# jianwang-mpi/GlobalEgoMocap

Hardware: AMD Instinct MI355X
Metric: optimised windows/sec (10-frame, 15-joint) (higher is better)
Workload: dtype f32

## Files before the change

### globalegomocap_amd/csrc/lbfgs.hip

```cpp
#include "gem_internal.h"

namespace gem {

typedef float f32x4 __attribute__((ext_vector_type(4)));

enum { PH_INIT = 0, PH_BRACKET = 1, PH_ZOOM = 2, PH_DONE = 3 };
static_assert(PH_DONE == 3, "Workspace::done_phase (gem_internal.h) names this value for the fused compaction of gemm_rows.h");

struct AdvArgs {
    LbfgsState* state;
    const double* f;
    double* trace;
    const float* gnew;
    float *x, *d, *g, *gp, *bg0, *bg1, *trial, *S, *Y;
    uint16_t* trial_b;
    int* phase_arr;
    const int* slot_of;
    int *next_perm, *next_slot_of, *next_count;
    SlabSrc gslab;
    unsigned long long* clk;
    int Dp, hist_cap;
    gem_lbfgs_opts o;
};

__device__ __forceinline__ double cubic_interpolate(double x1, double f1, double g1, double x2, double f2, double g2,
                                                    bool has_bounds, double lo, double hi) {
    if (!has_bounds) {
        lo = x1 <= x2 ? x1 : x2;
        hi = x1 <= x2 ? x2 : x1;
    }
    const double d1 = g1 + g2 - 3.0 * (f1 - f2) / (x1 - x2);
    const double d2s = d1 * d1 - g1 * g2;
    if (d2s >= 0.0) {
        const double d2 = sqrt(d2s);
        double m;
        if (x1 <= x2) m = x2 - (x2 - x1) * ((g2 + d2 - d1) / (g2 - g1 + 2.0 * d2));
        else m = x1 - (x1 - x2) * ((g1 + d2 - d1) / (g1 - g2 + 2.0 * d2));
        double r = (m > lo) ? m : lo;
        if (!(m == m)) r = m;
        double q = (r < hi) ? r : hi;
        if (!(r == r)) q = r;
        return q;
    }
    return (lo + hi) / 2.0;
}

template <int NT>
struct BlockRed {
    double* red;
    int parity;
    __device__ __forceinline__ double sum(double v) {
        double w[1] = {v};
        sumN<1>(w);
        return w[0];
    }
    template <int N>
    __device__ __forceinline__ void sumN(double (&v)[N]) {
#pragma unroll
        for (int n = 0; n < N; ++n) v[n] = wave_sum_dpp(v[n]);
        if (NT == 64) return;
        double* r = red + 12 * parity;
        parity ^= 1;
        if ((threadIdx.x & 63) == 0) {
#pragma unroll
            for (int n = 0; n < N; ++n) r[(threadIdx.x >> 6) * 3 + n] = v[n];
        }
        __syncthreads();
#pragma unroll
        for (int n = 0; n < N; ++n) v[n] = r[n] + r[3 + n] + r[6 + n] + r[9 + n];
    }
    __device__ __forceinline__ double max(double v) {
        v = wave_max_dpp(v);
        if (NT == 64) return v;
        double* r = red + 12 * parity;
        parity ^= 1;
        if ((threadIdx.x & 63) == 0) r[(threadIdx.x >> 6) * 3] = v;
        __syncthreads();
        return nan_max(nan_max(nan_max(r[0], r[3]), r[6]), r[9]);
    }
};

template <int EPT, int NT, bool FULL, bool HB>
__device__ __forceinline__ void lbfgs_advance_body(const AdvArgs& a) {
    __shared__ double red[24];
    __shared__ double ro_s[MAX_HIST];
    __shared__ double cadj_s[MAX_HIST];
    __shared__ double al_s[MAX_HIST];
    const int b = blockIdx.x, tid = threadIdx.x;
    LbfgsState* sp = a.state + b;
    int phase = sp->phase;
    const int gslot = a.slot_of ? a.slot_of[b] : b;
    const double f_new = a.f[b];
    if (phase == PH_DONE) return;
    BlockRed<NT> R{red, 0};
#ifdef GEM_LB_PROBE
    unsigned long long ts[10];
#pragma unroll
    for (int i = 0; i < 10; ++i) ts[i] = 0ull;
#define LB_PROBE(n) do { if (a.clk) ts[n] = wall_clock64(); } while (0)
#else
#define LB_PROBE(n) do { } while (0)
#endif
    LB_PROBE(0);
    const int hmask = a.hist_cap - 1;
    const gem_lbfgs_opts& o = a.o;
    const int Dp = a.Dp;
    const size_t off = (size_t)b * Dp;

    int n_iter = sp->n_iter, evals = sp->evals, ls_iter = sp->ls_iter, ls_evals = sp->ls_evals, max_ls = sp->max_ls;
    int first_bracket = sp->first_bracket, ls_done = sp->ls_done, insuf = sp->insuf, low = sp->low, high = sp->high;
    int hist_count = sp->hist_count, hist_start = sp->hist_start;
    double loss = sp->loss, prev_loss = sp->prev_loss, t = sp->t, gtd = sp->gtd, d_norm = sp->d_norm, H_diag = sp->H_diag;
    double t_prev = sp->t_prev, f_prev = sp->f_prev, gtd_prev = sp->gtd_prev;
    double br_t[2] = {sp->br_t[0], sp->br_t[1]}, br_f[2] = {sp->br_f[0], sp->br_f[1]};
    double br_gtd[2] = {sp->br_gtd[0], sp->br_gtd[1]};
    static_assert(MAX_HIST <= NT, "one ring scalar per thread");

    if (a.trace && tid == 0) a.trace[b] = f_new;
    if (f_new != f_new && tid == 0) sp->nan_seen = 1;
    const float* gsrc = a.gnew + (size_t)gslot * Dp;
    float gn[EPT], xv[EPT], dv[EPT], gcur[EPT], yv[EPT], sv[EPT];
    bool have_x = false, have_d = false;
#pragma unroll
    for (int i = 0; i < EPT; ++i) xv[i] = dv[i] = gcur[i] = yv[i] = sv[i] = 0.f;
    auto load = [&](const float* p, float (&v)[EPT]) {
        if constexpr (EPT % 4 == 0) {
#pragma unroll
            for (int i = 0; i < EPT / 4; ++i) {
                const int e = (tid + NT * i) * 4;
                f32x4 w = {0.f, 0.f, 0.f, 0.f};
                if (FULL || e < Dp) w = *reinterpret_cast<const f32x4*>(p + off + e);
                v[4 * i] = w[0]; v[4 * i + 1] = w[1]; v[4 * i + 2] = w[2]; v[4 * i + 3] = w[3];
            }
        } else {
#pragma unroll
            for (int i = 0; i < EPT; ++i) { const int e = tid + NT * i; v[i] = (FULL || e < Dp) ? p[off + e] : 0.f; }
        }
    };
    auto store = [&](float* p, const float (&v)[EPT]) {
        if constexpr (EPT % 4 == 0) {
#pragma unroll
            for (int i = 0; i < EPT / 4; ++i) {
                const int e = (tid + NT * i) * 4;
                const f32x4 w = {v[4 * i], v[4 * i + 1], v[4 * i + 2], v[4 * i + 3]};
                if (FULL || e < Dp) *reinterpret_cast<f32x4*>(p + off + e) = w;
            }
        } else {
#pragma unroll
            for (int i = 0; i < EPT; ++i) { const int e = tid + NT * i; if (FULL || e < Dp) p[off + e] = v[i]; }
        }
    };
    auto hload = [&](const float* base, int slot, float (&v)[EPT]) {
        const size_t eo = ((size_t)b * a.hist_cap + slot) * Dp;
        if constexpr (!HB) { load(base + eo - off, v); }
        else {
            const uint16_t* q = reinterpret_cast<const uint16_t*>(base) + eo;
            if constexpr (EPT % 4 == 0) {
#pragma unroll
                for (int i = 0; i < EPT / 4; ++i) {
                    const int e = (tid + NT * i) * 4;
                    typedef unsigned int u2 __attribute__((ext_vector_type(2)));
                    u2 w = {0u, 0u};
                    if (FULL || e < Dp) w = *reinterpret_cast<const u2*>(q + e);
                    v[4 * i] = __builtin_bit_cast(float, w[0] << 16); v[4 * i + 1] = __builtin_bit_cast(float, w[0] & 0xFFFF0000u);
                    v[4 * i + 2] = __builtin_bit_cast(float, w[1] << 16); v[4 * i + 3] = __builtin_bit_cast(float, w[1] & 0xFFFF0000u);
                }
            } else {
#pragma unroll
                for (int i = 0; i < EPT; ++i) { const int e = tid + NT * i; v[i] = (FULL || e < Dp) ? __builtin_bit_cast(float, (unsigned)q[e] << 16) : 0.f; }
            }
        }
    };
    auto hstore = [&](float* base, int slot, const float (&v)[EPT]) {
        const size_t eo = ((size_t)b * a.hist_cap + slot) * Dp;
        if constexpr (!HB) { store(base + eo - off, v); }
        else {
            uint16_t* q = reinterpret_cast<uint16_t*>(base) + eo;
            if constexpr (EPT % 4 == 0) {
#pragma unroll
                for (int i = 0; i < EPT / 4; ++i) {
                    const int e = (tid + NT * i) * 4;
                    typedef __bf16 bf4 __attribute__((ext_vector_type(4)));
                    const bf4 w = __builtin_convertvector(f32x4{v[4 * i], v[4 * i + 1], v[4 * i + 2], v[4 * i + 3]}, bf4);
                    if (FULL || e < Dp) *reinterpret_cast<bf4*>(q + e) = w;
                }
            } else {
#pragma unroll
                for (int i = 0; i < EPT; ++i) { const int e = tid + NT * i; if (FULL || e < Dp) q[e] = (uint16_t)(__builtin_bit_cast(unsigned int, (float)(__bf16)v[i]) >> 16); }
            }
        }
    };
    auto store_trial = [&](const float (&v)[EPT]) {
        if (!a.trial_b) store(a.trial, v);
        if (a.trial_b) {
            uint16_t* p = a.trial_b + off;
            if constexpr (EPT % 4 == 0) {
#pragma unroll
                for (int i = 0; i < EPT / 4; ++i) {
                    const int e = (tid + NT * i) * 4;
                    typedef __bf16 bf4 __attribute__((ext_vector_type(4)));
                    const bf4 w = __builtin_convertvector(f32x4{v[4 * i], v[4 * i + 1], v[4 * i + 2], v[4 * i + 3]}, bf4);
                    if (FULL || e < Dp) *reinterpret_cast<bf4*>(p + e) = w;
                }
            } else {
#pragma unroll
                for (int i = 0; i < EPT; ++i) {
                    const int e = tid + NT * i;
                    if (FULL || e < Dp) p[e] = (uint16_t)(__builtin_bit_cast(unsigned int, (float)(__bf16)v[i]) >> 16);
                }
            }
        }
    };
    auto copy = [&](float* dst, const float* src) {
        float tmp[EPT];
        load(src, tmp);
        store(dst, tmp);
    };
    auto dot = [&](const float (&u)[EPT], const float (&v)[EPT]) {
        float p = 0.f;
#pragma unroll
        for (int i = 0; i < EPT; ++i) p += u[i] * v[i];
        return R.sum((double)p);
    };
    auto maxabs = [&](const float (&u)[EPT], float scale) {
        float p = 0.f;
#pragma unroll
        for (int i = 0; i < EPT; ++i) { const float w = fabsf(u[i] * scale); p = (w > p || w != w) ? w : p; }
        return R.max((double)p);
    };
    LB_PROBE(1);
    double ro_v = 0.0, cadj_v = 0.0;
    auto request_rest = [&]() {
        if (tid < a.hist_cap) { ro_v = sp->ro[tid]; cadj_v = sp->cadj[tid]; }
        if (phase != PH_INIT) { load(a.d, dv); load(a.x, xv); have_d = have_x = true; }
    };
    if (a.gslab.base) {
        int nslab;
        size_t stride;
        slab_layout(a.gslab, nslab, stride);
        const float* gs = a.gslab.base + (size_t)gslot * Dp;
#pragma unroll
        for (int i = 0; i < EPT; ++i) gn[i] = 0.f;
        for (int z0 = 0; z0 < nslab; z0 += 8) {
            float t[8][EPT];
#pragma unroll
            for (int k = 0; k < 8; ++k) load(gs + (size_t)min(z0 + k, nslab - 1) * stride - off, t[k]);
            if (z0 == 0) request_rest();
#pragma unroll
            for (int k = 0; k < 8; ++k)
                if (z0 + k < nslab) {
#pragma unroll
                    for (int i = 0; i < EPT; ++i) gn[i] += t[k][i];
                }
        }
        if (nslab <= 0) request_rest();
    } else {
        load(gsrc - off, gn);
        request_rest();
    }
    if (tid < a.hist_cap) { ro_s[tid] = ro_v; cadj_s[tid] = cadj_v; }
    __syncthreads();
    float* BG[2] = {a.bg0, a.bg1};

    bool do_zoom_head = false, do_ls_end = false, do_start_iter = false, finished = false, emit = false;
    bool have_ys = false;

    LB_PROBE(2);
    if (phase == PH_INIT) {
        loss = f_new;
        evals = 1;
        n_iter = 0;
        store(a.g, gn);
#pragma unroll
        for (int i = 0; i < EPT; ++i) gcur[i] = gn[i];
        if (maxabs(gn, 1.f) <= o.tol_grad) finished = true;
        else do_start_iter = true;
    } else {
        const double gtd_new = dot(gn, dv);
        if (phase == PH_BRACKET) {
            if (!first_bracket) ls_iter++;
            first_bracket = 0;
            bool enter_zoom = false;
            if (ls_iter < max_ls) {
                const bool c1 = f_new > (loss + o.c1 * t * gtd) || (ls_iter > 1 && f_new >= f_prev);
                const bool c2 = fabs(gtd_new) <= -o.c2 * gtd;
                const bool c3 = gtd_new >= 0.0;
                if (c1 || (!c2 && c3)) {
                    br_t[0] = t_prev; br_t[1] = t;
                    br_f[0] = f_prev; br_f[1] = f_new;
                    br_gtd[0] = gtd_prev; br_gtd[1] = gtd_new;
                    copy(a.bg0, a.gp);
                    store(a.bg1, gn);
                    ls_done = 0;
                    enter_zoom = true;
                } else if (c2) {
                    br_t[0] = br_t[1] = t;
                    br_f[0] = br_f[1] = f_new;
                    br_gtd[0] = br_gtd[1] = gtd_new;
                    store(a.bg0, gn);
                    ls_done = 1;
                    enter_zoom = true;
                } else {
                    const double lo_b = t + 0.01 * (t - t_prev), hi_b = t * 10.0;
                    const double t_next = cubic_interpolate(t_prev, f_prev, gtd_prev, t, f_new, gtd_new, true, lo_b, hi_b);
                    t_prev = t; f_prev = f_new; gtd_prev = gtd_new;
                    store(a.gp, gn);
                    t = t_next;
                    emit = true;
                }
            } else {
                br_t[0] = 0.0; br_t[1] = t;
                br_f[0] = loss; br_f[1] = f_new;
                br_gtd[0] = gtd; br_gtd[1] = gtd_new;
                copy(a.bg0, a.g);
                store(a.bg1, gn);
                ls_done = 0;
                enter_zoom = true;
            }
            if (enter_zoom) {
                insuf = 0;
                if (br_f[0] <= br_f[1]) { low = 0; high = 1; } else { low = 1; high = 0; }
                do_zoom_head = true;
            }
        } else {
            ls_iter++;
            if (f_new > (loss + o.c1 * t * gtd) || f_new >= br_f[low]) {
                br_t[high] = t; br_f[high] = f_new; br_gtd[high] = gtd_new;
                store(BG[high], gn);
                if (br_f[0] <= br_f[1]) { low = 0; high = 1; } else { low = 1; high = 0; }
            } else {
                if (fabs(gtd_new) <= -o.c2 * gtd) {
                    ls_done = 1;
                } else if (gtd_new * (br_t[high] - br_t[low]) >= 0.0) {
                    br_t[high] = br_t[low]; br_f[high] = br_f[low]; br_gtd[high] = br_gtd[low];
                    copy(BG[high], BG[low]);
                }
                br_t[low] = t; br_f[low] = f_new; br_gtd[low] = gtd_new;
                store(BG[low], gn);
            }
            do_zoom_head = true;
        }
    }

    LB_PROBE(3);
    if (do_zoom_head) {
        if (ls_done || ls_iter >= max_ls) {
            do_ls_end = true;
        } else if (fabs(br_t[1] - br_t[0]) * d_norm < o.ls_tol_change) {
            do_ls_end = true;
        } else {
            double tn = cubic_interpolate(br_t[0], br_f[0], br_gtd[0], br_t[1], br_f[1], br_gtd[1], false, 0.0, 0.0);
            const double hi = br_t[0] > br_t[1] ? br_t[0] : br_t[1];
            const double lo = br_t[0] > br_t[1] ? br_t[1] : br_t[0];
            const double eps = 0.1 * (hi - lo);
            const double m1 = hi - tn, m2 = tn - lo;
            if ((m1 < m2 ? m1 : m2) < eps) {
                if (insuf || tn >= hi || tn <= lo) {
                    tn = (fabs(tn - hi) < fabs(tn - lo)) ? hi - eps : lo + eps;
                    insuf = 0;
                } else {
                    insuf = 1;
                }
            } else {
                insuf = 0;
            }
            t = tn;
            phase = PH_ZOOM;
            emit = true;
        }
    }

    LB_PROBE(4);
    if (do_ls_end) {
        __syncthreads();
        t = br_t[low];
        loss = br_f[low];
        float bl[EPT], gold[EPT];
        load(BG[low], bl);
        load(a.g, gold);
        const float tf = (float)t;
#pragma unroll
        for (int i = 0; i < EPT; ++i) {
            xv[i] = xv[i] + tf * dv[i];
            yv[i] = bl[i] - gold[i];
            sv[i] = dv[i] * tf;
            gcur[i] = bl[i];
        }
        store(a.x, xv);
        store(a.g, bl);
        evals += ls_evals;
        const double gmax = maxabs(bl, 1.f);
        const double dmax = maxabs(sv, 1.f);
        if (n_iter == o.max_iter || evals >= o.max_eval || gmax <= o.tol_grad || dmax <= o.tol_change ||
            fabs(loss - prev_loss) < o.tol_change) {
            finished = true;
        } else {
            do_start_iter = true;
            have_ys = true;
        }
    }

    LB_PROBE(5);
    bool full_path = false;
    if (do_start_iter) {
        n_iter++;
        if (n_iter == 1) {
#pragma unroll
            for (int i = 0; i < EPT; ++i) dv[i] = -gcur[i];
            H_diag = 1.0;
        } else {
            (void)have_ys;
            auto ring_slot = [&](int k) { return (hist_start + k) & hmask; };
            float sprev[EPT];
            const bool has_prev = hist_count >= 1;
            if (has_prev) hload(a.S, ring_slot(hist_count - 1), sprev);
            double r3[3] = {0.0, 0.0, 0.0};
            {
                float p0 = 0.f, p1 = 0.f, p2 = 0.f;
#pragma unroll
                for (int i = 0; i < EPT; ++i) {
                    p0 += yv[i] * sv[i];
                    p1 += yv[i] * yv[i];
                    if (has_prev) p2 += sprev[i] * yv[i];
                }
                r3[0] = (double)p0; r3[1] = (double)p1; r3[2] = (double)p2;
            }
            R.template sumN<3>(r3);
            full_path = true;
            LB_PROBE(6);
            const double ys = r3[0];
            const int limit = o.history < a.hist_cap ? o.history : a.hist_cap;
            if (ys > 1e-10) {
                const int prev_slot = (hist_start + hist_count - 1) & hmask;
                if (hist_count == limit) {
                    hist_start = (hist_start + 1) & hmask;
                    hist_count--;
                }
                const int slot = (hist_start + hist_count) & hmask;
                hstore(a.Y, slot, yv);
                hstore(a.S, slot, sv);
                const bool link = has_prev && hist_count >= 1;
                hist_count++;
                H_diag = ys / r3[1];
                if (tid == 0) {
                    ro_s[slot] = 1.0 / ys; sp->ro[slot] = 1.0 / ys;
                    if (link) { cadj_s[prev_slot] = r3[2]; sp->cadj[prev_slot] = r3[2]; }
                }
                __syncthreads();
            }
            float q[EPT];
#pragma unroll
            for (int i = 0; i < EPT; ++i) q[i] = -gcur[i];
            const int hc = hist_count, np2 = (hc + 1) / 2;
            float sXa[EPT], yXa[EPT], sXb[EPT], yXb[EPT], sZa[EPT], yZa[EPT], sZb[EPT], yZb[EPT];
            auto clampk = [&](int k) { return k < 0 ? 0 : (k >= hc ? hc - 1 : k); };
            auto ld2 = [&](int kA, int kB, float (&sA)[EPT], float (&yA)[EPT], float (&sB)[EPT], float (&yB)[EPT]) {
                hload(a.S, ring_slot(clampk(kA)), sA); hload(a.Y, ring_slot(clampk(kA)), yA);
                hload(a.S, ring_slot(clampk(kB)), sB); hload(a.Y, ring_slot(clampk(kB)), yB);
            };
            auto dstep1 = [&](int kA, float (&sA)[EPT], float (&yA)[EPT], float (&sB)[EPT], float (&yB)[EPT]) {
                const int kB = kA - 1;
                const bool vB = kB >= 0;
                const int slA = (hist_start + kA) & hmask, slB = (hist_start + clampk(kB)) & hmask;
                double r2[2];
                {
                    float pa = 0.f, pb = 0.f;
#pragma unroll
                    for (int i = 0; i < EPT; ++i) { pa += sA[i] * q[i]; pb += sB[i] * q[i]; }
                    r2[0] = (double)pa; r2[1] = (double)pb;
                }
                R.template sumN<2>(r2);
                const double alA = r2[0] * ro_s[slA];
                const double alB = vB ? (r2[1] - (double)(float)alA * cadj_s[slB]) * ro_s[slB] : 0.0;
                if (tid == 0) { al_s[kA] = alA; if (vB) al_s[kB] = alB; }
                const float fa = (float)alA, fb = (float)alB;
#pragma unroll
                for (int i = 0; i < EPT; ++i) q[i] -= fa * yA[i] + fb * yB[i];
            };
            auto dstep2 = [&](int kA, float (&sA)[EPT], float (&yA)[EPT], float (&sB)[EPT], float (&yB)[EPT]) {
                const int kB = kA + 1;
                const bool vB = kB < hc;
                const int slA = (hist_start + kA) & hmask, slB = (hist_start + clampk(kB)) & hmask;
                double r2[2];
                {
                    float pa = 0.f, pb = 0.f;
#pragma unroll
                    for (int i = 0; i < EPT; ++i) { pa += yA[i] * q[i]; pb += yB[i] * q[i]; }
                    r2[0] = (double)pa; r2[1] = (double)pb;
                }
                R.template sumN<2>(r2);
                const float cfA = (float)(al_s[kA] - r2[0] * ro_s[slA]);
                const float cfB = vB ? (float)(al_s[clampk(kB)] - (r2[1] + (double)cfA * cadj_s[slA]) * ro_s[slB]) : 0.f;
#pragma unroll
                for (int i = 0; i < EPT; ++i) q[i] += cfA * sA[i] + cfB * sB[i];
            };
            if (hc > 0) ld2(hc - 1, hc - 2, sXa, yXa, sXb, yXb);
            for (int p2 = 0; p2 < np2; p2 += 2) {
                const int kA = hc - 1 - 2 * p2;
                ld2(kA - 2, kA - 3, sZa, yZa, sZb, yZb);
                dstep1(kA, sXa, yXa, sXb, yXb);
                ld2(kA - 4, kA - 5, sXa, yXa, sXb, yXb);
                if (p2 + 1 < np2) dstep1(kA - 2, sZa, yZa, sZb, yZb);
            }
            __syncthreads();
            const float hd = (float)H_diag;
#pragma unroll
            for (int i = 0; i < EPT; ++i) q[i] *= hd;
            if (hc > 0) ld2(0, 1, sXa, yXa, sXb, yXb);
            for (int p2 = 0; p2 < np2; p2 += 2) {
                const int kA = 2 * p2;
                ld2(kA + 2, kA + 3, sZa, yZa, sZb, yZb);
                dstep2(kA, sXa, yXa, sXb, yXb);
                ld2(kA + 4, kA + 5, sXa, yXa, sXb, yXb);
                if (p2 + 1 < np2) dstep2(kA + 2, sZa, yZa, sZb, yZb);
            }
#pragma unroll
            for (int i = 0; i < EPT; ++i) dv[i] = q[i];
        }
        LB_PROBE(7);
        have_d = true;
        store(a.d, dv);
        prev_loss = loss;
        if (n_iter == 1) {
            float p = 0.f;
#pragma unroll
            for (int i = 0; i < EPT; ++i) p += fabsf(gcur[i]);
            const double l1 = R.sum((double)p);
            const double inv = 1.0 / l1;
            t = (inv < 1.0 ? inv : 1.0) * o.lr;
        } else {
            t = o.lr;
        }
        gtd = dot(gcur, dv);
        if (gtd > -o.tol_change) {
            finished = true;
        } else {
            d_norm = maxabs(dv, 1.f);
            max_ls = o.max_eval - evals;
            ls_iter = 0;
            ls_evals = 0;
            t_prev = 0.0; f_prev = loss; gtd_prev = gtd;
            store(a.gp, gcur);
            phase = PH_BRACKET;
            first_bracket = 1;
            emit = true;
        }
    }

    LB_PROBE(8);
    if (finished) {
        phase = PH_DONE;
        if (!have_x) load(a.x, xv);
        store_trial(xv);
    } else if (emit) {
        if (!have_x) load(a.x, xv);
        if (!have_d) load(a.d, dv);
        const float tf = (float)t;
        float tr[EPT];
#pragma unroll
        for (int i = 0; i < EPT; ++i) tr[i] = xv[i] + tf * dv[i];
        store_trial(tr);
        ls_evals++;
    }
    if (tid == 0) {
        if (a.next_count && phase != PH_DONE) {
            const int slot = atomicAdd(a.next_count, 1);
            a.next_perm[slot] = b;
            a.next_slot_of[b] = slot;
        }
        if (a.phase_arr) a.phase_arr[b] = phase;
        sp->phase = phase; sp->n_iter = n_iter; sp->evals = evals; sp->ls_iter = ls_iter; sp->ls_evals = ls_evals;
        sp->max_ls = max_ls; sp->first_bracket = first_bracket; sp->ls_done = ls_done; sp->insuf = insuf;
        sp->low = low; sp->high = high; sp->hist_count = hist_count; sp->hist_start = hist_start;
        sp->loss = loss; sp->prev_loss = prev_loss; sp->t = t; sp->gtd = gtd; sp->d_norm = d_norm; sp->H_diag = H_diag;
        sp->t_prev = t_prev; sp->f_prev = f_prev; sp->gtd_prev = gtd_prev;
        sp->br_t[0] = br_t[0]; sp->br_t[1] = br_t[1]; sp->br_f[0] = br_f[0]; sp->br_f[1] = br_f[1];
        sp->br_gtd[0] = br_gtd[0]; sp->br_gtd[1] = br_gtd[1];
    }
    LB_PROBE(9);
#ifdef GEM_LB_PROBE
    if (a.clk && tid == 0 && full_path) {
        unsigned long long prev = ts[0];
#pragma unroll
        for (int i = 1; i < 10; ++i)
            if (ts[i]) { atomicAdd(a.clk + i, ts[i] - prev); prev = ts[i]; }
        atomicAdd(a.clk + 30, (unsigned long long)hist_count);
        atomicAdd(a.clk + 31, 1ull);
    }
#endif
    (void)full_path;
#undef LB_PROBE
}

template <int EPT, bool FULL, bool HB = false>
__global__ __launch_bounds__(256) void lbfgs_advance_kernel(AdvArgs a) { lbfgs_advance_body<EPT, 256, FULL, HB>(a); }

__global__ void lbfgs_init_kernel(LbfgsState* st, int* __restrict__ phase_arr, const float* __restrict__ trial, float* __restrict__ x, int B,
                                  int Dp) {
    const size_t i = (size_t)blockIdx.x * blockDim.x + threadIdx.x;
    if (i < (size_t)B * Dp) x[i] = trial[i];
    if (i < (size_t)B) {
        phase_arr[i] = PH_INIT;
        LbfgsState* s = st + i;
        s->phase = PH_INIT; s->n_iter = 0; s->evals = 0; s->ls_iter = 0; s->ls_evals = 0; s->max_ls = 0;
        s->first_bracket = 0; s->ls_done = 0; s->insuf = 0; s->low = 0; s->high = 1; s->hist_count = 0; s->hist_start = 0;
        s->nan_seen = 0;
        s->loss = 0; s->prev_loss = 0; s->t = 0; s->gtd = 0; s->d_norm = 0; s->H_diag = 1;
        s->t_prev = 0; s->f_prev = 0; s->gtd_prev = 0;
        s->br_t[0] = s->br_t[1] = 0; s->br_f[0] = s->br_f[1] = 0; s->br_gtd[0] = s->br_gtd[1] = 0;
    }
}

__global__ void lbfgs_stats_kernel(const LbfgsState* st, gem_window_stats* out, int B) {
    const int i = blockIdx.x * blockDim.x + threadIdx.x;
    if (i >= B) return;
    out[i].n_iter = st[i].n_iter;
    out[i].func_evals = st[i].evals;
    out[i].final_loss = (float)st[i].loss;
    out[i].status = (st[i].phase == PH_DONE ? 1 : 0) | (st[i].nan_seen ? 2 : 0);
}

static AdvArgs make_args(gem_handle* h, const gem_lbfgs_opts& o) {
    Workspace& w = h->ws;
    AdvArgs a;
    a.state = w.state; a.f = w.f; a.gnew = w.dz;
    a.trace = (w.round >= 0 && w.round < TRACE_ROUNDS) ? w.trace + (size_t)w.round * w.Bmax : nullptr;
    a.x = w.x; a.d = w.d; a.g = w.g; a.gp = w.gp; a.bg0 = w.bg0; a.bg1 = w.bg1; a.trial = w.trial; a.S = w.S; a.Y = w.Y;
    a.trial_b = h->precision == GEM_PRECISION_BF16 ? w.trial_b : nullptr;
    a.phase_arr = w.phase;
    a.slot_of = w.dyn ? w.slot_of : nullptr;
    a.next_perm = w.dyn ? w.next_perm : nullptr; a.next_slot_of = w.dyn ? w.next_slot_of : nullptr; a.next_count = w.dyn ? w.next_count : nullptr;
    a.gslab = w.dyn ? w.grad_slab : SlabSrc{};
    a.clk = w.lbfgs_clk;
    a.Dp = h->Dp; a.hist_cap = w.hist_cap; a.o = o;
    return a;
}

int launch_lbfgs_init(gem_handle* h, int B, const gem_lbfgs_opts& o, hipStream_t s) {
    (void)o;
    const size_t n = (size_t)B * h->Dp;
    hipLaunchKernelGGL(lbfgs_init_kernel, dim3((unsigned)((n + 255) / 256)), dim3(256), 0, s, h->ws.state, h->ws.phase, h->ws.trial, h->ws.x,
                       B, h->Dp);
    GEM_HIP(hipGetLastError());
    return 0;
}

int launch_lbfgs_advance(gem_handle* h, int B, const gem_lbfgs_opts& o, hipStream_t s) {
    AdvArgs a = make_args(h, o);
    Profile::Rec rec;
    const bool prof = h->prof.on;
    if (prof) {
        GEM_HIP(hipEventCreate(&rec.a)); GEM_HIP(hipEventCreate(&rec.b));
        rec.family = 2; rec.flops = 0;
        GEM_HIP(hipEventRecord(rec.a, s));
    }
    const int ept = (h->Dp + 255) / 256;
    typedef void (*kern_t)(AdvArgs);
    kern_t kern = nullptr;
    if (ept <= 1) kern = lbfgs_advance_kernel<1, false>;
    else if (ept <= 2) kern = lbfgs_advance_kernel<2, false>;
    else if (ept <= 4) kern = lbfgs_advance_kernel<4, false>;
    else if (h->Dp == 2048 && h->precision == GEM_PRECISION_BF16) kern = lbfgs_advance_kernel<8, true, true>;
    else if (h->Dp == 2048) kern = lbfgs_advance_kernel<8, true>;
    else if (ept <= 8) kern = lbfgs_advance_kernel<8, false>;
    else if (ept <= 16) kern = lbfgs_advance_kernel<16, false>;
    else { set_error("latent_dim > 4096 is not supported by the L-BFGS kernel"); return 1; }
    note_kernel(h, reinterpret_cast<const void*>(kern));
    hipLaunchKernelGGL(kern, dim3(B), dim3(256), 0, s, a);
    GEM_HIP(hipGetLastError());
    if (prof) { GEM_HIP(hipEventRecord(rec.b, s)); h->prof.recs.push_back(rec); }
    commit_kernel_names(h, prof ? 2 : -1);
    return 0;
}

__global__ __launch_bounds__(1024) void compact_kernel(const int* __restrict__ phase_arr, int B, int T, int* __restrict__ perm,
                                                       int* __restrict__ slot_of, int* __restrict__ n_active, int force_all,
                                                       int* __restrict__ log_slot, int zero_after) {
    __shared__ int wsum[16];
    const int tid = threadIdx.x, lane = tid & 63, wave = tid >> 6;
    const int E = (B + 1023) >> 10, b0 = tid * E;
    unsigned long long mask = 0ull;
    for (int e = 0; e < E; ++e) {
        const int b = b0 + e;
        if (b < B && (force_all || phase_arr[b] != PH_DONE)) mask |= 1ull << e;
    }
    const int cnt = __popcll(mask);
    int incl = cnt;
#pragma unroll
    for (int d = 1; d < 64; d <<= 1) {
        const int v = __shfl_up(incl, d);
        if (lane >= d) incl += v;
    }
    if (lane == 63) wsum[wave] = incl;
    __syncthreads();
    int woff = 0, total = 0;
#pragma unroll
    for (int i = 0; i < 16; ++i) { if (i < wave) woff += wsum[i]; total += wsum[i]; }
    int pa = woff + incl - cnt;
    int pi = total + (b0 - pa);
    for (int e = 0; e < E; ++e) {
        const int b = b0 + e;
        if (b >= B) break;
        if ((mask >> e) & 1ull) { perm[pa] = b; slot_of[b] = pa++; }
        else { perm[pi] = b; slot_of[b] = pi++; }
    }
    if (tid == 0) { n_active[0] = total; n_active[1] = total * T; *log_slot = total; }
    if (tid < zero_after) log_slot[1 + tid] = 0;
}

int launch_compact(gem_handle* h, int B, int force_all, hipStream_t s, int zero_after) {
    Workspace& w = h->ws;
    if (B > 65536) { set_error("compact: more than 65536 windows per call"); return 1; }
    if (zero_after < 0 || zero_after > 1024 || (w.log_pos % N_LOG) + zero_after >= N_LOG) { set_error("compact: bad counter range"); return 1; }
    hipLaunchKernelGGL(compact_kernel, dim3(1), dim3(1024), 0, s, w.phase, B, h->T, w.perm, w.slot_of, w.n_active, force_all,
                       w.n_log + (w.log_pos % N_LOG), zero_after);
    GEM_HIP(hipGetLastError());
    w.cur_log = w.log_pos++;
    return 0;
}

int launch_lbfgs_stats(gem_handle* h, int B, gem_window_stats* out, hipStream_t s) {
    hipLaunchKernelGGL(lbfgs_stats_kernel, dim3((B + 255) / 256), dim3(256), 0, s, h->ws.state, out, B);
    GEM_HIP(hipGetLastError());
    return 0;
}

}
```

### globalegomocap_amd/csrc/tail.hip

```cpp
#include <algorithm>

#include "energy_device.h"

namespace gem {

typedef float f32x16 __attribute__((ext_vector_type(16)));
typedef float f32x4 __attribute__((ext_vector_type(4)));

__device__ __forceinline__ float bf16_round(float x) {
    const __bf16 b = (__bf16)x;
    return (float)b;
}

constexpr int TAIL_WAVES = 8;
constexpr int TAIL_THREADS = TAIL_WAVES * 64;
constexpr int TAIL_WAVES_SHARED = 4;

constexpr int TAIL_ROWS = 16;

template <int W>
__device__ __forceinline__ void tail_prefetch_first(const TailLayerDev L, f32x4 (&dst)[4]) {
    const int lane = threadIdx.x & 63, wave = __builtin_amdgcn_readfirstlane(threadIdx.x >> 6);
    const int c = lane & 15, q = lane >> 4;
    const int n0 = wave * 16;
    if (n0 >= L.N) return;
    const f32x4* p = reinterpret_cast<const f32x4*>(L.w4) + (size_t)q * L.N + n0 + c;
#pragma unroll
    for (int g = 0; g < 4; ++g) dst[g] = p[(size_t)(4 * g) * L.N];
}

template <int W, int NT, typename Epi>
__device__ __forceinline__ void tail_gemm_nt(const float* in, int ld_in, const float* zero_line, const TailLayerDev L,
                                             const TailLayerDev next, bool has_next, int T, int R, f32x4 (&bpre)[4], Epi epi,
                                             int c0 = 0, bool use_pre = true) {
    const int tid = threadIdx.x, lane = tid & 63, wave = __builtin_amdgcn_readfirstlane(tid >> 6);
    const int fr = lane & 15, fq = lane >> 4;
    const int kb = L.K / 64, nblk = 3 * kb;
    const f32x4* W4 = reinterpret_cast<const f32x4*>(L.w4);
    constexpr int TS = 16 * W;
    const int n0 = wave * 16 + c0;
    if (n0 >= L.N) {
        if (has_next) tail_prefetch_first<W>(next, bpre);
        return;
    }
    const int row = fr;
    const int t_row = row % T;
    const bool row_ok = row < R;
    float bv[NT];
    f32x4 acc[NT];
#pragma unroll
    for (int i = 0; i < NT; ++i) {
        bv[i] = L.bias ? L.bias[n0 + TS * i + fr] : 0.f;
        acc[i] = f32x4{0.f, 0.f, 0.f, 0.f};
    }
    const f32x4* pB = W4 + (size_t)fq * L.N + n0 + fr;
    const int strideB = 16 * L.N;
    const int a_own = row * ld_in + 4 * fq;
    const int a_zero = (int)(zero_line - in) + 4 * fq;
    const bool ok_m = row_ok && t_row >= 1, ok_p = row_ok && t_row + 1 < T;
#define TAIL_LOAD_B(blk_, dst_)                                                                        \
    {                                                                                                  \
        const f32x4* p_ = pB + (size_t)(blk_) * strideB;                                               \
        _Pragma("unroll") for (int i = 0; i < NT; ++i)                                                 \
            _Pragma("unroll") for (int g = 0; g < 4; ++g) dst_[i][g] = p_[(size_t)(4 * g) * L.N + TS * i]; \
    }
#define TAIL_LOAD_A(blk_, dst_)                                                                        \
    {                                                                                                  \
        const int tap_ = ((blk_) >= kb) + ((blk_) >= 2 * kb), k0_ = ((blk_) - tap_ * kb) * 64;         \
        const bool ok_ = tap_ == 0 ? ok_m : (tap_ == 1 ? row_ok : ok_p);                               \
        const float* arow_ = in + (ok_ ? a_own + (tap_ - 1) * ld_in + k0_ : a_zero);                   \
        _Pragma("unroll") for (int g = 0; g < 4; ++g) dst_[g] = *reinterpret_cast<const f32x4*>(arow_ + 16 * g); \
    }
#define TAIL_COMPUTE(a_, b_)                                                                           \
    {                                                                                                  \
        _Pragma("unroll") for (int g = 0; g < 4; ++g) {                                                \
            _Pragma("unroll") for (int i = 0; i < NT; ++i) acc[i] = __builtin_amdgcn_mfma_f32_16x16x4f32(a_[g].x, b_[i][g].x, acc[i], 0, 0, 0); \
            _Pragma("unroll") for (int i = 0; i < NT; ++i) acc[i] = __builtin_amdgcn_mfma_f32_16x16x4f32(a_[g].y, b_[i][g].y, acc[i], 0, 0, 0); \
            _Pragma("unroll") for (int i = 0; i < NT; ++i) acc[i] = __builtin_amdgcn_mfma_f32_16x16x4f32(a_[g].z, b_[i][g].z, acc[i], 0, 0, 0); \
            _Pragma("unroll") for (int i = 0; i < NT; ++i) acc[i] = __builtin_amdgcn_mfma_f32_16x16x4f32(a_[g].w, b_[i][g].w, acc[i], 0, 0, 0); \
        }                                                                                              \
    }
    f32x4 b0[NT][4], b1[NT][4], a0[4], a1[4];
    TAIL_LOAD_B(0, b0);
    if (use_pre) {
#pragma unroll
        for (int g = 0; g < 4; ++g) b0[0][g] = bpre[g];
    }
    TAIL_LOAD_A(0, a0);
    const int npairs = nblk / 2;
#define TAIL_INTERLEAVE()                                                                                          \
    {                                                                                                              \
        _Pragma("unroll") for (int i_ = 0; i_ < 4 * NT; ++i_) { __builtin_amdgcn_sched_group_barrier(0x008, 2, 0); __builtin_amdgcn_sched_group_barrier(0x020, 1, 0); } \
        _Pragma("unroll") for (int i_ = 0; i_ < 4; ++i_) { __builtin_amdgcn_sched_group_barrier(0x008, 2 * NT, 0); __builtin_amdgcn_sched_group_barrier(0x100, 1, 0); } \
    }
    for (int p = 0; p < npairs; ++p) {
        const int blk = 2 * p;
        TAIL_LOAD_B(blk + 1, b1);
        TAIL_LOAD_A(blk + 1, a1);
        TAIL_COMPUTE(a0, b0);
        TAIL_INTERLEAVE();
        __builtin_amdgcn_sched_barrier(0);
        const int nxt = min(blk + 2, nblk - 1);
        TAIL_LOAD_B(nxt, b0);
        TAIL_LOAD_A(nxt, a0);
        TAIL_COMPUTE(a1, b1);
        TAIL_INTERLEAVE();
        __builtin_amdgcn_sched_barrier(0);
    }
#undef TAIL_INTERLEAVE
    if (nblk & 1) TAIL_COMPUTE(a0, b0);
    if (has_next) tail_prefetch_first<W>(next, bpre);
#undef TAIL_LOAD_A
#undef TAIL_LOAD_B
#undef TAIL_COMPUTE
#pragma unroll
    for (int i = 0; i < NT; ++i) epi(acc[i], 4 * fq, n0 + TS * i + fr, bv[i]);
}

template <int W, typename Epi>
__device__ __forceinline__ void tail_gemm(const float* in, int ld_in, const float* zero_line, const TailLayerDev L,
                                          const TailLayerDev next, bool has_next, int T, int R, f32x4 (&bpre)[4], Epi epi) {
    if constexpr (W == TAIL_WAVES_SHARED) {
        if (L.N > 32 * W) {
            tail_gemm_nt<W, 2>(in, ld_in, zero_line, L, next, false, T, R, bpre, epi);
            tail_gemm_nt<W, 2>(in, ld_in, zero_line, L, next, has_next, T, R, bpre, epi, 32 * W, false);
        } else if (L.N > 16 * W) tail_gemm_nt<W, 2>(in, ld_in, zero_line, L, next, has_next, T, R, bpre, epi);
        else tail_gemm_nt<W, 1>(in, ld_in, zero_line, L, next, has_next, T, R, bpre, epi);
    } else {
        if (L.N > 32 * W) tail_gemm_nt<W, 4>(in, ld_in, zero_line, L, next, has_next, T, R, bpre, epi);
        else if (L.N > 16 * W) tail_gemm_nt<W, 2>(in, ld_in, zero_line, L, next, has_next, T, R, bpre, epi);
        else tail_gemm_nt<W, 1>(in, ld_in, zero_line, L, next, has_next, T, R, bpre, epi);
    }
}

template <int NL, int W>
__global__ __launch_bounds__(64 * W, W == TAIL_WAVES_SHARED ? 3 : 2) void decoder_tail_kernel(TailArgs a) {
    constexpr int THREADS = 64 * W;
    constexpr bool TIGHT = W == TAIL_WAVES_SHARED;
    constexpr int STAGE_U = 2048 / THREADS;
    constexpr int PRE_E = TAIL_THREADS / THREADS;
    extern __shared__ __attribute__((aligned(16))) float lds[];
    const int tid = threadIdx.x, lane = tid & 63, wave = __builtin_amdgcn_readfirstlane(tid >> 6);
    const int T = a.e.T;
    int probe = 0;
#define TAIL_PROBE()                                                                                   \
    if (a.dbg_ts && blockIdx.x == 0 && tid == 0) {                                                     \
        a.dbg_ts[2 * probe] = clock64();                                                               \
        a.dbg_ts[2 * probe + 1] = wall_clock64();                                                      \
        ++probe;                                                                                       \
    }
    const int w0 = blockIdx.x * a.G;
    const int B = a.e.n_dev ? *a.e.n_dev : a.B;
    if (w0 >= B) return;
    const int nwin = min(a.G, B - w0);
    const int R = nwin * T;
    const size_t row0 = (size_t)w0 * T;

    {
        const int K0 = a.fwd[0].K, q4 = K0 / 4, n4 = (TIGHT ? a.rows : TAIL_ROWS) * q4;
        float* dst = lds + a.off_act[0];
        if (a.in_slab.base) {
            int nslab;
            size_t stride;
            slab_layout(a.in_slab, nslab, stride);
            for (int u = 0; u < STAGE_U; ++u) {
                const int i = tid + u * THREADS, r = i / q4, c = (i - r * q4) * 4;
                if (i >= n4) break;
                f32x4 v = {0.f, 0.f, 0.f, 0.f};
                if (r < R) {
                    const float* p = a.in_slab.base + (row0 + r) * K0 + c;
                    for (int z0 = 0; z0 < nslab; z0 += 8) {
                        f32x4 t[8];
#pragma unroll
                        for (int k = 0; k < 8; ++k) t[k] = *reinterpret_cast<const f32x4*>(p + (size_t)min(z0 + k, nslab - 1) * stride);
#pragma unroll
                        for (int k = 0; k < 8; ++k)
                            if (z0 + k < nslab) v += t[k];
                    }
                    v += *reinterpret_cast<const f32x4*>(a.in_bias + (r % T) * a.in_bias_ld + c);
#pragma unroll
                    for (int q = 0; q < 4; ++q) v[q] = v[q] > 0.f ? v[q] : v[q] * LEAKY_SLOPE;
                }
                *reinterpret_cast<f32x4*>(dst + r * a.ld_act[0] + c) = v;
            }
        } else {
            f32x4 v[STAGE_U];
#pragma unroll
            for (int u = 0; u < STAGE_U; ++u) {
                const int i = tid + u * THREADS, r = i / q4, c = (i - r * q4) * 4;
                v[u] = f32x4{0.f, 0.f, 0.f, 0.f};
                if (i < n4 && r < R) v[u] = *reinterpret_cast<const f32x4*>(a.a_in + (row0 + r) * K0 + c);
            }
#pragma unroll
            for (int u = 0; u < STAGE_U; ++u) {
                const int i = tid + u * THREADS, r = i / q4, c = (i - r * q4) * 4;
                if (i < n4) *reinterpret_cast<f32x4*>(dst + r * a.ld_act[0] + c) = v[u];
            }
        }
        if (tid < 64) lds[a.off_zero + tid] = 0.f;
    }
    float pre_x0[PRE_E], pre_mb = 0.f;
    int pre_par = 0, pre_ch[PRE_E];
#pragma unroll
    for (int k = 0; k < PRE_E; ++k) { pre_x0[k] = 0.f; pre_ch[k] = -1; }
    static_assert(MAXJ * MAXJ <= TAIL_THREADS && MAXJ <= 64, "the children table is parked by PRE_E passes of the workgroup");
    const bool pre_on = a.G == 1 && !a.forward_only && T * a.e.J * 3 <= TAIL_THREADS;
    if (pre_on) {
        const int J = a.e.J, n = T * J * 3, bw = a.e.perm ? a.e.perm[w0] : w0;
#pragma unroll
        for (int k = 0; k < PRE_E; ++k) {
            const int e = tid + k * THREADS;
            if (e < n) pre_x0[k] = a.e.X0[(size_t)bw * n + e];
            if (e < J * MAXJ) pre_ch[k] = a.e.children[e];
        }
        if (tid < J) { pre_mb = a.e.mean_bone[(size_t)bw * J + tid]; pre_par = a.e.parents[tid]; }
    }
    TAIL_PROBE();
    __syncthreads();
    TAIL_PROBE();

    f32x4 bpre[4];
    tail_prefetch_first<W>(a.fwd[0], bpre);
#pragma unroll
    for (int i = 0; i < NL; ++i) {
        const bool last = (i + 1 == NL);
        float* out = lds + a.off_act[i + 1];
        const int ldo = a.ld_act[i + 1];
        float* Xp = last ? a.Xp : nullptr;
        const TailLayerDev nxt = !last ? a.fwd[i + 1 < NL ? i + 1 : i] : a.bwd[NL - 1];
        tail_gemm<W>(lds + a.off_act[i], a.ld_act[i], lds + a.off_zero, a.fwd[i], nxt, !last || !a.forward_only, T, R, bpre,
                  [&](const f32x4& acc, int r0, int col, float bv) {
#pragma unroll
                      for (int e = 0; e < 4; ++e) {
                          float v = acc[e] + bv;
                          if (!last) v = v > 0.f ? v : v * LEAKY_SLOPE;
                          if (!TIGHT || r0 + e < a.rows) out[(r0 + e) * ldo + col] = v;
                          if (Xp && r0 + e < R) Xp[(row0 + r0 + e) * PAD + col] = v;
                      }
                  });
        if (i == 0 && pre_on) {
            const int J = a.e.J, n = T * J * 3;
            float* pre = lds + a.off_pre;
            int* prei = reinterpret_cast<int*>(pre + n + J);
#pragma unroll
            for (int k = 0; k < PRE_E; ++k) {
                const int e = tid + k * THREADS;
                if (e < n) pre[e] = pre_x0[k];
                if (e < J * MAXJ) prei[J + e] = pre_ch[k];
            }
            if (tid < J) { pre[n + tid] = pre_mb; prei[tid] = pre_par; }
        }
        __syncthreads();
        TAIL_PROBE();
    }
    if (a.forward_only) return;

    float* g_cur = lds + a.off_g[0];
    float* g_nxt = lds + a.off_g[1];
    if (a.G == 1) {
        float* scr = lds + a.off_escr;
        const int J = a.e.J, n = T * J * 3;
        const float* pre = lds + a.off_pre;
        const int* prei = reinterpret_cast<const int*>(pre + n + J);
        if (T == 10 && J == 15)
            energy_window<true, THREADS, 10, 15>(a.e, a.e.perm ? a.e.perm[w0] : w0, tid, lds + a.off_act[NL], a.ld_act[NL], scr,
                                                      scr + a.escr, scr + 2 * a.escr, scr + 3 * a.escr, g_cur, a.ld_g, a.fwd[NL - 1].N,
                                                      nullptr, pre_on ? pre : nullptr, pre_on ? pre + n : nullptr, pre_on ? prei : nullptr,
                                                      pre_on ? prei + J : nullptr);
        else
            energy_window<true, THREADS>(a.e, a.e.perm ? a.e.perm[w0] : w0, tid, lds + a.off_act[NL], a.ld_act[NL], scr,
                                              scr + a.escr, scr + 2 * a.escr, scr + 3 * a.escr, g_cur, a.ld_g, a.fwd[NL - 1].N,
                                              nullptr, pre_on ? pre : nullptr, pre_on ? pre + n : nullptr, pre_on ? prei : nullptr,
                                              pre_on ? prei + J : nullptr);
    } else if (wave < nwin) {
        float* scr = lds + a.off_escr + wave * 4 * a.escr;
        energy_window<false>(a.e, a.e.perm ? a.e.perm[w0 + wave] : w0 + wave, lane,
                             lds + a.off_act[NL] + wave * T * a.ld_act[NL], a.ld_act[NL], scr, scr + a.escr,
                             scr + 2 * a.escr, scr + 3 * a.escr, g_cur + wave * T * a.ld_g, a.ld_g, a.fwd[NL - 1].N);
    }
    __syncthreads();
    TAIL_PROBE();

#pragma unroll
    for (int i = NL - 1; i >= 0; --i) {
        const float* act = lds + a.off_act[i];
        const int lda = a.ld_act[i];
        const int ldg = a.ld_g;
        float* gout = a.g_out;
        uint16_t* gout_b = a.g_out_b;
        const int K0 = a.fwd[0].K;
        tail_gemm<W>(g_cur, a.ld_g, lds + a.off_zero, a.bwd[i], a.bwd[i > 0 ? i - 1 : 0], i > 0, T, R, bpre,
                  [&](const f32x4& acc, int r0, int col, float) {
#pragma unroll
                      for (int e = 0; e < 4; ++e) {
                          const int row = r0 + e;
                          const float v = (i > 0 || a.mask_first) ? acc[e] * (act[row * lda + col] > 0.f ? 1.f : LEAKY_SLOPE) : acc[e];
                          if (i > 0) { if (!TIGHT || row < a.rows) g_nxt[row * ldg + col] = v; }
                          else if (row < R) {
                              if (gout_b) gout_b[(row0 + row) * K0 + col] = (uint16_t)(__builtin_bit_cast(unsigned int, bf16_round(v)) >> 16);
                              else gout[(row0 + row) * K0 + col] = v;
                          }
                      }
                  });
        __syncthreads();
        TAIL_PROBE();
        float* t = g_cur; g_cur = g_nxt; g_nxt = t;
    }
#undef TAIL_PROBE
}

size_t plan_tail(const std::vector<Layer>& dec, int start, int T, int J, TailArgs* out, bool shared) {
    const int n = (int)dec.size() - start;
    if (start < 0 || n < 1 || n > TAIL_MAX_LAYERS || T > TAIL_ROWS) return 0;
    for (int i = start; i < (int)dec.size(); ++i) {
        const int K = dec[i].K, N = dec[i].N;
        auto ok = [](int v) { return v == 64 || v == 128 || v == 256 || v == 512; };
        if (!ok(K) || !ok(N)) return 0;
    }
    TailArgs a{};
    a.n = n;
    a.mask_first = start > 0;
    a.G = TAIL_ROWS / T;
    if (shared && a.G != 1) return 0;
    a.waves = shared ? TAIL_WAVES_SHARED : TAIL_WAVES;
    a.rows = shared ? a.G * T : TAIL_ROWS;
    const int rows = a.rows;
    int off = 0, maxg = 0;
    for (int i = 0; i <= n; ++i) {
        const int width = i == 0 ? dec[start].K : dec[start + i - 1].N;
        a.off_act[i] = off;
        a.ld_act[i] = width + 4;
        off += rows * (width + 4);
        if (i >= 1 && width > maxg) maxg = width;
    }
    a.ld_g = maxg + 4;
    a.off_g[0] = off; off += rows * a.ld_g;
    a.off_g[1] = off; off += rows * a.ld_g;
    a.escr = (T * J * 3 + 3) / 4 * 4;
    a.off_red = off;
    a.off_escr = off;
    off += a.G * 4 * a.escr;
    a.off_zero = off;
    off += 64;
    a.off_pre = off;
    if (a.G == 1) off += (T * J * 3 + 2 * J + J * MAXJ + 3) / 4 * 4;
    if (out) *out = a;
    return (size_t)off * sizeof(float);
}

template <int NL, int W>
static void launch_tail_as(gem_handle* h, const TailArgs& a, int wgs, size_t lds_bytes, hipStream_t s) {
    note_kernel(h, reinterpret_cast<const void*>(decoder_tail_kernel<NL, W>));
    hipLaunchKernelGGL((decoder_tail_kernel<NL, W>), dim3(wgs), dim3(64 * W), lds_bytes, s, a);
}

template <int W>
static int launch_tail_w(gem_handle* h, const TailArgs& a, int wgs, size_t lds_bytes, hipStream_t s) {
    switch (a.n) {
        case 1: launch_tail_as<1, W>(h, a, wgs, lds_bytes, s); break;
        case 2: launch_tail_as<2, W>(h, a, wgs, lds_bytes, s); break;
        case 3: launch_tail_as<3, W>(h, a, wgs, lds_bytes, s); break;
        case 4: launch_tail_as<4, W>(h, a, wgs, lds_bytes, s); break;
        case 5: launch_tail_as<5, W>(h, a, wgs, lds_bytes, s); break;
        case 6: launch_tail_as<6, W>(h, a, wgs, lds_bytes, s); break;
        default: set_error("launch_tail: unsupported number of fused layers"); return 1;
    }
    return 0;
}

static bool tail_can_share_cu(const std::vector<Layer>& dec, int start, int T, int J) {
    const size_t bytes = plan_tail(dec, start, T, J, nullptr, true);
    if (!bytes || 3 * bytes > 160 * 1024) return false;
    for (int i = start; i < (int)dec.size(); ++i)
        if (dec[i].N > 64 * TAIL_WAVES_SHARED || dec[i].K > 64 * TAIL_WAVES_SHARED) return false;
    return true;
}

size_t plan_tail_for(const gem_handle* h, const std::vector<Layer>& dec, int start, int wgs, TailArgs* out) {
    bool shared = wgs > h->n_cu && tail_can_share_cu(dec, start, h->T, h->J);
    if (const char* f = dev_env("GEM_TAIL_WAVES")) shared = atoi(f) == TAIL_WAVES_SHARED && tail_can_share_cu(dec, start, h->T, h->J);
    return plan_tail(dec, start, h->T, h->J, out, shared);
}

int tail_cap_workgroups(const gem_handle* h, const std::vector<Layer>& dec, int start) {
    if (const char* f = dev_env("GEM_TAIL_CAP")) return atoi(f) * h->n_cu;
    return (tail_can_share_cu(dec, start, h->T, h->J) ? 10 : 5) * h->n_cu;
}

int launch_tail(gem_handle* h, const TailArgs& a, size_t lds_bytes, hipStream_t s) {
    static PerDeviceOnce attr_once;
    if (attr_once.need(h->cfg.device)) {
        const void* ks[] = {reinterpret_cast<const void*>(decoder_tail_kernel<1, 8>), reinterpret_cast<const void*>(decoder_tail_kernel<2, 8>),
                            reinterpret_cast<const void*>(decoder_tail_kernel<3, 8>), reinterpret_cast<const void*>(decoder_tail_kernel<4, 8>),
                            reinterpret_cast<const void*>(decoder_tail_kernel<5, 8>), reinterpret_cast<const void*>(decoder_tail_kernel<6, 8>),
                            reinterpret_cast<const void*>(decoder_tail_kernel<1, 4>), reinterpret_cast<const void*>(decoder_tail_kernel<2, 4>),
                            reinterpret_cast<const void*>(decoder_tail_kernel<3, 4>), reinterpret_cast<const void*>(decoder_tail_kernel<4, 4>),
                            reinterpret_cast<const void*>(decoder_tail_kernel<5, 4>), reinterpret_cast<const void*>(decoder_tail_kernel<6, 4>)};
        for (const void* k : ks) GEM_HIP(hipFuncSetAttribute(k, hipFuncAttributeMaxDynamicSharedMemorySize, 160 * 1024));
    }
    Profile::Rec rec;
    const bool prof = h->prof.on;
    if (prof) {
        GEM_HIP(hipEventCreate(&rec.a)); GEM_HIP(hipEventCreate(&rec.b));
        rec.family = 1;
        double per_window = 0.0;
        for (int i = 0; i < a.n; ++i) per_window += 2.0 * 3.0 * a.fwd[i].K * a.fwd[i].N * a.e.T;
        if (!a.forward_only) per_window *= 2.0;
        rec.flops = per_window * a.B;
        if (h->ws.dyn) { rec.log_idx = h->ws.cur_log; rec.flops_per_window = per_window; }
        GEM_HIP(hipEventRecord(rec.a, s));
    }
    const int wgs = (a.B + a.G - 1) / a.G;
    if (a.waves != TAIL_WAVES && a.waves != TAIL_WAVES_SHARED) { set_error("launch_tail: the arguments do not come from plan_tail"); return 1; }
    if (a.waves == TAIL_WAVES_SHARED ? launch_tail_w<TAIL_WAVES_SHARED>(h, a, wgs, lds_bytes, s) : launch_tail_w<TAIL_WAVES>(h, a, wgs, lds_bytes, s))
        return 1;
    GEM_HIP(hipGetLastError());
    if (prof) { GEM_HIP(hipEventRecord(rec.b, s)); h->prof.recs.push_back(rec); }
    commit_kernel_names(h, prof ? 1 : -1);
    return 0;
}

}
```

Baseline: 32020.

## Cache newest L-BFGS history pairs in registers and batch tail slab-sum loads

Adds a ring-kernel variant of the L-BFGS advance for Dp=2048 fp32 when the batch fits in the CU count. It preloads the newest nine S/Y history pairs into registers so the two-loop recursion reads them without going back to global memory, and it falls back to global loads for older entries. Separately, the tail kernel's input staging is specialised for slab counts of 2, 4 and 8 so that all slab and bias loads are issued before any reduction, which raises memory-level parallelism. The cost is much higher register pressure in the ring kernel, with possible spills, and extra template instantiations.

After: 30280. 5.4% lower.

```diff
diff --git a/globalegomocap_amd/csrc/lbfgs.hip b/globalegomocap_amd/csrc/lbfgs.hip
--- a/globalegomocap_amd/csrc/lbfgs.hip
+++ b/globalegomocap_amd/csrc/lbfgs.hip
@@ -80,8 +80,10 @@
     }
 };
 
-template <int EPT, int NT, bool FULL, bool HB>
+constexpr int RING_PAIRS = 9;
+template <int EPT, int NT, bool FULL, bool HB, bool RING = false>
 __device__ __forceinline__ void lbfgs_advance_body(const AdvArgs& a) {
+    static_assert(!RING || !HB, "the register copy of the ring is bitwise the ring only when the ring is fp32");
     __shared__ double red[24];
     __shared__ double ro_s[MAX_HIST];
     __shared__ double cadj_s[MAX_HIST];
@@ -230,6 +232,9 @@
     };
     LB_PROBE(1);
     double ro_v = 0.0, cadj_v = 0.0;
+    constexpr int RC = RING ? RING_PAIRS : 1;
+    float cS[RC][EPT], cY[RC][EPT];
+    const int ring_n = hist_count < RING_PAIRS ? hist_count : RING_PAIRS;
     auto request_rest = [&]() {
         if (tid < a.hist_cap) { ro_v = sp->ro[tid]; cadj_v = sp->cadj[tid]; }
         if (phase != PH_INIT) { load(a.d, dv); load(a.x, xv); have_d = have_x = true; }
@@ -260,6 +265,15 @@
     }
     if (tid < a.hist_cap) { ro_s[tid] = ro_v; cadj_s[tid] = cadj_v; }
     __syncthreads();
+    if constexpr (RING) {
+        const int newest = hist_count > 0 ? hist_count - 1 : 0;
+#pragma unroll
+        for (int c = 0; c < RING_PAIRS; ++c) {
+            const int slot = (hist_start + newest - (c < newest ? c : newest)) & hmask;
+            hload(a.S, slot, cS[c]);
+            hload(a.Y, slot, cY[c]);
+        }
+    }
     float* BG[2] = {a.bg0, a.bg1};
 
     bool do_zoom_head = false, do_ls_end = false, do_start_iter = false, finished = false, emit = false;
@@ -413,7 +427,14 @@
             auto ring_slot = [&](int k) { return (hist_start + k) & hmask; };
             float sprev[EPT];
             const bool has_prev = hist_count >= 1;
-            if (has_prev) hload(a.S, ring_slot(hist_count - 1), sprev);
+            if constexpr (RING) {
+                if (has_prev) {
+#pragma unroll
+                    for (int i = 0; i < EPT; ++i) sprev[i] = cS[0][i];
+                }
+            } else {
+                if (has_prev) hload(a.S, ring_slot(hist_count - 1), sprev);
+            }
             double r3[3] = {0.0, 0.0, 0.0};
             {
                 float p0 = 0.f, p1 = 0.f, p2 = 0.f;
@@ -429,6 +450,7 @@
             full_path = true;
             LB_PROBE(6);
             const double ys = r3[0];
+            int pushed = 0;
             const int limit = o.history < a.hist_cap ? o.history : a.hist_cap;
             if (ys > 1e-10) {
                 const int prev_slot = (hist_start + hist_count - 1) & hmask;
@@ -441,6 +463,7 @@
                 hstore(a.S, slot, sv);
                 const bool link = has_prev && hist_count >= 1;
                 hist_count++;
+                pushed = 1;
                 H_diag = ys / r3[1];
                 if (tid == 0) {
                     ro_s[slot] = 1.0 / ys; sp->ro[slot] = 1.0 / ys;
@@ -454,9 +477,30 @@
             const int hc = hist_count, np2 = (hc + 1) / 2;
             float sXa[EPT], yXa[EPT], sXb[EPT], yXb[EPT], sZa[EPT], yZa[EPT], sZb[EPT], yZb[EPT];
             auto clampk = [&](int k) { return k < 0 ? 0 : (k >= hc ? hc - 1 : k); };
+            auto fetch = [&](int k, float (&s)[EPT], float (&y)[EPT]) {
+                k = clampk(k);
+                if constexpr (RING) {
+                    const int c = hc - 1 - k - pushed;
+                    if (c < 0) {
+#pragma unroll
+                        for (int i = 0; i < EPT; ++i) { s[i] = sv[i]; y[i] = yv[i]; }
+                        return;
+                    }
+                    if (c < ring_n) {
+#pragma unroll
+                        for (int j = 0; j < RING_PAIRS; ++j)
+                            if (c == j) {
+#pragma unroll
+                                for (int i = 0; i < EPT; ++i) { s[i] = cS[j][i]; y[i] = cY[j][i]; }
+                            }
+                        return;
+                    }
+                }
+                hload(a.S, ring_slot(k), s); hload(a.Y, ring_slot(k), y);
+            };
             auto ld2 = [&](int kA, int kB, float (&sA)[EPT], float (&yA)[EPT], float (&sB)[EPT], float (&yB)[EPT]) {
-                hload(a.S, ring_slot(clampk(kA)), sA); hload(a.Y, ring_slot(clampk(kA)), yA);
-                hload(a.S, ring_slot(clampk(kB)), sB); hload(a.Y, ring_slot(clampk(kB)), yB);
+                fetch(kA, sA, yA);
+                fetch(kB, sB, yB);
             };
             auto dstep1 = [&](int kA, float (&sA)[EPT], float (&yA)[EPT], float (&sB)[EPT], float (&yB)[EPT]) {
                 const int kB = kA - 1;
@@ -588,12 +632,13 @@
         atomicAdd(a.clk + 31, 1ull);
     }
 #endif
-    (void)full_path;
+    (void)full_path; (void)cS; (void)cY; (void)ring_n;
 #undef LB_PROBE
 }
 
 template <int EPT, bool FULL, bool HB = false>
 __global__ __launch_bounds__(256) void lbfgs_advance_kernel(AdvArgs a) { lbfgs_advance_body<EPT, 256, FULL, HB>(a); }
+__global__ __launch_bounds__(256) void lbfgs_advance_ring_kernel(AdvArgs a) { lbfgs_advance_body<8, 256, true, false, true>(a); }
 
 __global__ void lbfgs_init_kernel(LbfgsState* st, int* __restrict__ phase_arr, const float* __restrict__ trial, float* __restrict__ x, int B,
                                   int Dp) {
@@ -655,12 +700,15 @@
         GEM_HIP(hipEventRecord(rec.a, s));
     }
     const int ept = (h->Dp + 255) / 256;
+    const char* ring_env = dev_env("GEM_LBFGS_RING_LDS");
+    const bool ring_off = ring_env && ring_env[0] == '0';
     typedef void (*kern_t)(AdvArgs);
     kern_t kern = nullptr;
     if (ept <= 1) kern = lbfgs_advance_kernel<1, false>;
     else if (ept <= 2) kern = lbfgs_advance_kernel<2, false>;
     else if (ept <= 4) kern = lbfgs_advance_kernel<4, false>;
     else if (h->Dp == 2048 && h->precision == GEM_PRECISION_BF16) kern = lbfgs_advance_kernel<8, true, true>;
+    else if (h->Dp == 2048 && B <= h->n_cu && !ring_off) kern = lbfgs_advance_ring_kernel;
     else if (h->Dp == 2048) kern = lbfgs_advance_kernel<8, true>;
     else if (ept <= 8) kern = lbfgs_advance_kernel<8, false>;
     else if (ept <= 16) kern = lbfgs_advance_kernel<16, false>;
diff --git a/globalegomocap_amd/csrc/tail.hip b/globalegomocap_amd/csrc/tail.hip
--- a/globalegomocap_amd/csrc/tail.hip
+++ b/globalegomocap_amd/csrc/tail.hip
@@ -1,4 +1,5 @@
 #include <algorithm>
+#include <type_traits>
 
 #include "energy_device.h"
 
@@ -163,7 +164,41 @@
             int nslab;
             size_t stride;
             slab_layout(a.in_slab, nslab, stride);
-            for (int u = 0; u < STAGE_U; ++u) {
+            bool staged = false;
+            if constexpr (!TIGHT) {
+                auto stage = [&](auto ns_c) {
+                    constexpr int NS = decltype(ns_c)::value;
+                    f32x4 t[STAGE_U][NS], bz[STAGE_U];
+#pragma unroll
+                    for (int u = 0; u < STAGE_U; ++u) {
+                        const int i = min(tid + u * THREADS, n4 - 1), r = i / q4, c = (i - r * q4) * 4, rc = min(r, R - 1);
+                        const float* p = a.in_slab.base + (row0 + rc) * K0 + c;
+#pragma unroll
+                        for (int k = 0; k < NS; ++k) t[u][k] = *reinterpret_cast<const f32x4*>(p + (size_t)k * stride);
+                        bz[u] = *reinterpret_cast<const f32x4*>(a.in_bias + (rc % T) * a.in_bias_ld + c);
+                    }
+#pragma unroll
+                    for (int u = 0; u < STAGE_U; ++u) {
+                        const int i = tid + u * THREADS, r = i / q4, c = (i - r * q4) * 4;
+                        f32x4 v = {0.f, 0.f, 0.f, 0.f};
+#pragma unroll
+                        for (int k = 0; k < NS; ++k) v += t[u][k];
+                        v += bz[u];
+#pragma unroll
+                        for (int q = 0; q < 4; ++q) v[q] = v[q] > 0.f ? v[q] : v[q] * LEAKY_SLOPE;
+                        if (r >= R) v = f32x4{0.f, 0.f, 0.f, 0.f};
+                        if (i < n4) *reinterpret_cast<f32x4*>(dst + r * a.ld_act[0] + c) = v;
+                    }
+                };
+                staged = true;
+                switch (nslab) {
+                    case 2: stage(std::integral_constant<int, 2>{}); break;
+                    case 4: stage(std::integral_constant<int, 4>{}); break;
+                    case 8: stage(std::integral_constant<int, 8>{}); break;
+                    default: staged = false;
+                }
+            }
+            for (int u = 0; u < STAGE_U && !staged; ++u) {
                 const int i = tid + u * THREADS, r = i / q4, c = (i - r * q4) * 4;
                 if (i >= n4) break;
                 f32x4 v = {0.f, 0.f, 0.f, 0.f};
```
